# rlglab/minizero

Measured on AMD Instinct MI355X. Metric: self-play leaf-evals/s (9x9 Go AlphaZero n=400), higher is better.
Workload: dtype f32; 1 GPU; BASELINE configs[1]: 9x9 Go AlphaZero, n=400, 6 blocks x 64 ch, 256 parallel games per GPU, synthetic fixed-weight net (seed 0), Dirichlet noise + random rotation + softmax-count moves (reference defaults); games_per_gpu=256, actor_num_simulation=400, pipeline_lanes=1, backend=nccl

## Files before the change

### include/mzgpu.h

```cpp
#ifndef MZGPU_H
#define MZGPU_H
#include <stddef.h>
#include <stdint.h>

#ifdef __cplusplus
extern "C" {
#endif

#define MZ_OK 0
#define MZ_ERR_ARG (-1)
#define MZ_ERR_DEVICE (-2)
#define MZ_ERR_STATE (-3)
#define MZ_ERR_CAPACITY (-4)

#define MZ_HOST 0
#define MZ_DEVICE 1

const char* mz_last_error(void);
int mz_device_count(void);
int mz_usable_cpus(void);

typedef struct mz_net_desc {
    char game_name[64];
    int num_input_channels, input_channel_height, input_channel_width;
// ... 136 lines not shown
int mz_env_legal_mask(const mz_env* e, uint8_t* out);
int mz_env_features(const mz_env* e, int rotation, float* out);
int mz_env_action_from_string(const mz_env* e, const char* action_string);
int mz_env_feature_bits(const mz_env* e, int rotation, uint32_t* out);
int mz_env_name(const mz_env* e, char* out, int cap);

int mz_godev_playout(int device, int board_size, float komi, const int* actions, int count, int root_prefix, const int* rots,
                     uint32_t* feat_out, uint8_t* legal_out, int* terminal_out, float* eval_out, int* player_out);
int mz_envdev_playout(int device, const char* game, int board_size, float komi, const int* actions, int count, int root_prefix, const int* rots,
                      uint32_t* feat_out, uint8_t* legal_out, int* terminal_out, float* eval_out, int* player_out);
int mz_envdev_playout_conf(int device, const char* conf, const int* actions, int count, int root_prefix, const int* rots,
                           uint32_t* feat_out, uint8_t* legal_out, int* terminal_out, float* eval_out, int* player_out);
int mz_sort_candidates(int device, const float* policy, int n, int* order_out);
int mz_invert_values_device(int device, const float* values, int n, float* out);
int mz_exp_tanh_device(int device, const float* x, int n, float* exp_out, float* tanh_out);

#ifdef __cplusplus
}
#endif
#endif
```

### minizero_amd/__init__.py

```python
from .lib import (MzError, NetDesc, SearchCfg, WorkerStats, Net, Pool, Worker, Env, DataLoader, load, lib_path, make_desc,
                  param_count, generate_weights, device_count, usable_cpus, godev_playout, envdev_playout, envdev_playout_conf, sort_candidates, invert_values_device, exp_tanh_device, read_pt, read_weight_file, read_weights_once, weight_file_reads, DESCS, CONFIGS)
```

### minizero_amd/csrc/net.h

```cpp
#pragma once
#include "common.h"
#include "game_kind.h"
#include <string>

namespace mz {

struct ConvLayer {
    int cin, cin_pad, cout, cout_pad;
    size_t w_off, b_off;
    size_t w4_off;
    size_t wq_off;
    int cq;
};

struct HeadOffsets {
    int pc;
    size_t pconv_w, pconv_b, pfc_wT, pfc_b, vconv_w, vconv_b, vfc1_wT, vfc1_b, vfc2_w, vfc2_b;
};

struct DiscreteHeadOffsets {
    int hc = 0, hidden = 0, size = 0;
    size_t conv_w = 0, conv_b = 0, fc1_wT = 0, fc1_b = 0, fc2_wT = 0, fc2_b = 0;
};
struct AtariLayers {
// ... 40 lines not shown
    int reload(const float* raw, size_t n);

    int forwardAZ(const float* d_feat, int B, float* d_policy, float* d_logit, float* d_value, bool in_bits = false);
    bool hasFusedTower();
    int initial(const float* d_feat, int B, float* d_policy, float* d_logit, float* d_value, float* d_hidden, const int* d_dst_idx);
    int recurrent(const float* d_hidden_src, const int* d_src_idx, const float* d_action_planes, const int* d_action_ids, int B, float* d_policy,
                  float* d_logit, float* d_value, float* d_reward, float* d_hidden_dst, const int* d_dst_idx);
    int forwardAZ_any(const float* feat, int B, float* policy, float* logit, float* value, int where);
    int initial_any(const float* feat, int B, float* policy, float* logit, float* value, float* hidden, int where);
    int recurrent_any(const float* hidden_in, const float* action, int B, float* policy, float* logit, float* value, float* reward, float* hidden_out,
                      int where);
    int simLaunch(Pool& pool, const GoDevView& gv, float* d_policy, float* d_logit, float* d_value, const uint8_t* d_rot, int sim0, int nsims,
                  bool* launched, const float* d_root_noise = nullptr, float noise_eps = 0.0f, int noise_kind = kNoiseDirichlet, const struct GumbelView* gum = nullptr,
                  int* d_start = nullptr, bool host_start = false);
    void allowTailHelp(bool on) { tail_help_ = on; }
    bool hasSimKernel(int board_n, int env_kind = kGo, int num_simulation = 0) const;
    bool hasSimKernelWide(int board_n, int env_kind, int num_simulation) const;
    bool simWidePlan(int board_n, int env_kind, int num_simulation, const HeadParams& hp, int channels, int W32, size_t leaf_bytes, size_t scratch_bytes, int* lf, size_t* lds,
                     size_t* tile_bytes_out) const;
    int simLaunchWide(const struct SimArgs& a, const GoDevView& gv, int max_depth, const uint8_t* d_rot, int sim0, int nsims, bool host_start, int lf, size_t lds, bool* launched);
    int uploadSimArgs(const struct SimArgs& a);
    int simLaunchMz(Pool& pool, float* d_hidden, int slots, const unsigned* d_root_feat, const unsigned long long* d_root_legal, const int* d_root_turn,
                    int num_players, float* d_policy, float* d_logit, float* d_value, float* d_reward, int sim0, int nsims, bool* launched,
                    const float* d_root_noise, float noise_eps, int noise_kind, const GumbelView* gum, int* d_start, bool host_start, bool root_given = false,
                    int pre_epoch = 0, bool noise_applied = false, const SimMzMode& mode = SimMzMode());
    int simPreEvalMz(int games, int max_depth, int s0, int R, int epoch, bool* launched, bool want_alt = true, bool pairs = false);
    int simPreEvalBatchMz(int games, int max_depth, int s0, int R, int epoch, bool* launched, int force_nl = 0, bool want_alt = false);
    bool hasPreBatch() const;
    bool pairsAvailable() const { return pair_ok_; }
    void pairTrouble() { pair_ok_ = false; }
// ... 98 lines not shown
```

### minizero_amd/csrc/sim.hip

```cpp
#include "sim_az_body.h"
#include "sim_mz_body.h"

namespace mz {

MZ_SPEC_WAYS_IS(16);

template <int H, int W, int CIN0_PAD, int CDYN_PAD, int CPAD>
__global__ __launch_bounds__(512) void sim_kernel_mz(const SimArgs* __restrict__ a_, int sim0, int nsims, int host_start, int pre_epoch)
{
    CSimArgs* a = (CSimArgs*)a_;
    extern __shared__ __attribute__((aligned(16))) float tiles[];
    const int g = blockIdx.x, tid = threadIdx.x, lane = tid & 63, wave = tid >> 6;
    constexpr int CM = CIN0_PAD > CDYN_PAD ? (CIN0_PAD > CPAD ? CIN0_PAD : CPAD) : (CDYN_PAD > CPAD ? CDYN_PAD : CPAD);
    constexpr int kTileFloats = kTowerTiles * CM * planeStride(H, W);
    double* rcp_w = reinterpret_cast<double*>(tiles + kTileFloats);
    const int rcp_n = a->rcp_n;
    for (int i = tid; i < rcp_n; i += 512) { rcp_w[i] = a->pv.rcp_tab[i]; }
    LdsCDouble* rcp_lds = (LdsCDouble*)rcp_w;
    const int tab_n = rcp_n - 2;
    double* sqrt_w = rcp_w + rcp_n;
    float* bias_w = reinterpret_cast<float*>(sqrt_w + tab_n);
    int* spec_w = reinterpret_cast<int*>(bias_w + tab_n + (tab_n & 1));
    for (int i = tid; i < tab_n; i += 512) { sqrt_w[i] = a->pv.sqrt_tab[i]; bias_w[i] = a->pv.bias_tab[i]; }
    if (!a->atari) {
// ... 380 lines not shown
    X(8, 8, 4, 64, kRulesOthello)    \
    X(8, 8, 4, 8, kRulesOthello)     \
    X(3, 3, 4, 16, kRulesTicTacToe)

__global__ void sim_prof_fold(unsigned long long* tail)
{
    if (threadIdx.x != 0 || blockIdx.x != 0) { return; }
    const unsigned long long n = tail[5];
    if (n > 0) {
        const unsigned long long start = tail[0];
        tail[8] += 1;
        tail[9] += tail[1] - start;
        tail[10] += tail[2] - start;
        tail[11] += tail[3] / n - start;
        tail[12] += tail[6] / n;
    }
    tail[0] = ~0ull; tail[1] = ~0ull; tail[2] = 0; tail[3] = 0; tail[5] = 0; tail[6] = 0;
    tail[4] = wall_clock64();
}

int Net::simProfBuffer(int games, unsigned long long** prof)
{
    if (sim_prof_.n == 0) {
        if (!sim_prof_.alloc(size_t(games) * 8 + kSimProfTail)) { setError("hipMalloc of the profile buffer failed"); return MZ_ERR_DEVICE; }
        MZ_HIP(hipMemsetAsync(sim_prof_.p, 0, sim_prof_.n * sizeof(unsigned long long), stream_));
    }
    hipLaunchKernelGGL(sim_prof_fold, dim3(1), dim3(1), 0, stream_, sim_prof_.p + sim_prof_.n - kSimProfTail);
    MZ_HIP(hipGetLastError());
    *prof = sim_prof_.p;
    return MZ_OK;
}

// ... 83 lines not shown
    {
        double tw = 0, hd = 0;
        for (size_t g = 0; g < G; ++g) { tw += double(h[g * 8 + 1]); hd += double(h[g * 8 + 2]); }
        const double ran = std::max(1.0, sims_all - skipped);
        fprintf(stderr, "[mz sim prof] terminal leaves: network skipped in %.0f of %.0f simulations (%.2f %%; the game with the most: %.2f %%) -> per simulation that ran them: tower %.2f us, heads %.2f us\n",
                skipped, sims_all, 100.0 * skipped / std::max(1.0, sims_all), 100.0 * skipped_max, tw / ran * 0.01, hd / ran * 0.01);
    }
    fprintf(stderr, "[mz sim prof] value first: %llu of %.0f simulations in the new order; %llu walks arrived at the previous simulation's leaf, %llu waited there (avg %.2f us); "
                    "%llu waits at the join in front of the leaf\n",
            tail[16], sims_all, tail[17], tail[18], double(tail[19]) / std::max(1.0, double(tail[18])) * 0.01, tail[20]);
    if (tail[8] > 0) {
        const double L = double(tail[8]), first = double(tail[9]) / L * 0.01, last = double(tail[10]) / L * 0.01, mean = double(tail[11]) / L * 0.01;
        const double helping = double(tail[12]) / L * 0.01;
        fprintf(stderr, "[mz sim prof] launches: %llu, avg per launch from the first game's start: first game done %.1f us, mean %.1f us, last %.1f us -> %.1f %% of the CU time idles at the end of a launch\n",
                tail[8], first, mean, last, 100.0 * (last - mean - helping) / std::max(1e-9, last));
        if (tail[13] > 0 || tail[15] > 0) {
            double tw = 0;
            for (size_t g = 0; g < G; ++g) { tw += double(h[g * 8 + 1]); }
            const double ran = sims_all - skipped, pn = double(tail[13]), pt = double(tail[14]);
            fprintf(stderr, "[mz sim prof] tail help: %.0f of the %.0f simulations that ran the network had a pair tower (%.2f %%): tower %.2f us with a helper, %.2f us alone; %llu games helped, "
                            "a CU helps for %.1f us per launch after its own game (%.1f %% of the launch)\n",
                    pn, ran, 100.0 * pn / std::max(1.0, ran), pt / std::max(1.0, pn) * 0.01, (tw - pt) / std::max(1.0, ran - pn) * 0.01, tail[15], helping,
                    100.0 * helping / std::max(1e-9, last));
        }
    }
}

static size_t simLdsBound(size_t tile_bytes, int n, int A, size_t head_floats)
{
    const size_t rcp_n = size_t(n) + 5, max_depth = size_t(n) + 3;
    return tile_bytes + rcp_n * (2 * sizeof(double) + sizeof(float)) + kSpecWords * sizeof(int) + (size_t(5) * (A + 1) + 26 + 18 * 12 + 2 * max_depth + 2 + head_floats) * sizeof(float) +
           size_t(kGoSeenCap) * sizeof(uint64_t);
}

int Net::uploadSimArgs(const SimArgs& a)
{
    static_assert(sizeof(SimArgs) % 4 == 0, "SimArgs is copied as words");
    if (sim_args_host_.size() != sizeof(SimArgs) || memcmp(sim_args_host_.data(), &a, sizeof(SimArgs)) != 0) {
// ... 397 lines not shown
```

### minizero_amd/csrc/sim_az_body.h

```cpp
#pragma once
#include "net.h"
#ifdef MZ_SIM_TPROF
__device__ unsigned long long g_tp[64];
__shared__ unsigned long long s_tp_prev;
__shared__ int s_tp_idx;
#define MZ_TPROF(slot)                                                                         \
    do {                                                                                       \
        if ((slot) == 3 && threadIdx.x == 0 && blockIdx.x == 0) {                              \
            const unsigned long long t_ = clock64();                                           \
            g_tp[s_tp_idx & 63] += t_ - s_tp_prev; s_tp_prev = t_; ++s_tp_idx;                 \
        }                                                                                      \
    } while (0)
#endif
#ifdef MZ_SIM_HPROF
#ifndef MZ_HPROF_BLOCK
#define MZ_HPROF_BLOCK 0
#endif
__device__ unsigned long long g_hp[16];
__shared__ unsigned long long s_hp_prev;
#define MZ_HPROF(k)                                                                                   \
    do {                                                                                              \
        if (threadIdx.x == 0 && blockIdx.x == MZ_HPROF_BLOCK) {                                       \
            const unsigned long long t_ = wall_clock64();                                             \
            if ((k) > 0) { g_hp[(k)] += t_ - s_hp_prev; } else { g_hp[15] += 1; }                     \
// ... 396 lines not shown
}
template <int WPE, bool BIGA = false, bool FP = BIGA>
__device__ __noinline__ void simHeads(CSimArgs* __restrict__ a, int g, int tid, float* tiles, const float* xtile, int xcs, int xpw, float* xchg)
{
    simHeadsImpl<WPE, BIGA, FP>(a, g, tid, tiles, xtile, xcs, xpw, xchg);
}

__device__ __forceinline__ bool simLeafTerminal(CSimArgs* __restrict__ a, const float* xchg)
{
    if (a->no_spec & 16) { return false; }
    const int A = a->gv.A;
    const SimXchg x{A + (A & 1)};
    return __builtin_amdgcn_readfirstlane(reinterpret_cast<const int*>(xchg + x.scalars())[6]) != 0;
}

constexpr int kSimProfTail = 24;
__device__ __forceinline__ void simProfEnter(unsigned long long* tail)
{
    atomicMin(tail + 0, wall_clock64() - tail[4]);
}
__device__ __forceinline__ void simProfExit(unsigned long long* tail)
{
    const unsigned long long t = wall_clock64() - tail[4];
    atomicMin(tail + 1, t);
    atomicMax(tail + 2, t);
    atomicAdd(tail + 3, t);
    atomicAdd(tail + 5, 1ull);
}

template <int H, int W, int CIN0_PAD, int CPAD, bool BF = false>
constexpr int simWavesPerEu() { return (!BF && H * W <= 64 && kTowerTiles * (CIN0_PAD > CPAD ? CIN0_PAD : CPAD) * planeStride(H, W) * 4 <= 76 * 1024) ? 4 : 2; }
// ... 9 lines not shown
#endif
    g = __builtin_amdgcn_readfirstlane(g);
    const GoDevView gv = simLeafView(ldc(&a->gv), xchg, g);
    return towerBody<H, W, CIN0_PAD, CPAD>(reinterpret_cast<const float*>(gv.feat), a->params, *(const TowerArgs*)&a->ta, nullptr, g, tid, tiles);
}

template <int H, int W>
__device__ __noinline__ const float* simTowerBf16(CSimArgs* __restrict__ a, int g, int tid, float* tiles, float* xchg)
{
    g = __builtin_amdgcn_readfirstlane(g);
    const GoDevView gv = simLeafView(ldc(&a->gv), xchg, g);
    return towerBodyBf16<H, W>(reinterpret_cast<const unsigned*>(gv.feat), a->wfrag, a->params, *(const TowerArgsBf16*)&a->tb, nullptr, g, tid,
                               reinterpret_cast<char*>(tiles));
}

template <int H, int W, int CIN0_PAD, int CPAD>
__device__ __noinline__ const float* simTowerPair(CSimArgs* __restrict__ a, int g, int tid, float* tiles, float* xchg, int seq, unsigned xseq, int* abort_lds)
{
    g = __builtin_amdgcn_readfirstlane(g);
    seq = __builtin_amdgcn_readfirstlane(seq);
    xseq = __builtin_amdgcn_readfirstlane(xseq);
    const GoDevView gv = simLeafView(ldc(&a->gv), xchg, g);
    const unsigned* bits = reinterpret_cast<const unsigned*>(gv.feat) + size_t(g) * gv.channels * gv.W32;
    unsigned* hb = a->help + size_t(g) * a->help_words;
    const int fw = gv.channels * gv.W32;
    if (tid < helpCmdUnits(fw)) {
        hpu4 u;
        u.x = bits[3 * tid];
        u.y = 3 * tid + 1 < fw ? bits[3 * tid + 1] : 0u;
        u.z = 3 * tid + 2 < fw ? bits[3 * tid + 2] : 0u;
        u.w = unsigned(seq);
        asm volatile("global_store_dwordx4 %0, %1, off" ::"v"(hb + kHpCmd + 4 * tid), "v"(u) : "memory");
    }
    HelpCtx c{hb, 0, xseq, abort_lds, a->err};
    return towerBodyPair<H, W, CIN0_PAD, CPAD>(bits, a->params, *(const TowerArgs*)&a->ta, tid, tiles, c);
}

template <int H, int W, int CIN0_PAD, int CPAD>
__device__ __noinline__ void simHelpTail(CSimArgs* __restrict__ a, int g, int tid, float* tiles, unsigned* bits, int nsims, int* s_help)
{
    g = __builtin_amdgcn_readfirstlane(g);
    nsims = __builtin_amdgcn_readfirstlane(nsims);
    const int lane = tid & 63, wave = __builtin_amdgcn_readfirstlane(tid >> 6);
    const int games = gridDim.x, words = a->help_words, min_left = a->help_min_left;
    const int fw = a->gv.channels * a->gv.W32, units = helpCmdUnits(fw);
    const unsigned myxcc = hpXccId();
    unsigned long long* ptail = a->prof ? a->prof + size_t(games) * 8 : nullptr;
    for (int round = 0; round < 64; ++round) {
        if (wave == 0) {
            unsigned key = ~0u;
            for (int o = (g & 7) + 8 * lane; o < games; o += 8 * 64) {
                const unsigned* ob = a->help + size_t(o) * words;
                const unsigned x = hpLoadU(ob + kHpXcc), p = hpLoadU(ob + kHpProgress), h = hpLoadU(ob + kHpHelper);
                const unsigned k = (p << 10) | unsigned(o);
                if (o != g && x == myxcc && h == 0u && int(p) + min_left <= nsims && k < key) { key = k; }
            }
            for (int o = 32; o > 0; o >>= 1) { const unsigned k2 = __shfl_xor(key, o); key = k2 < key ? k2 : key; }
            if (lane == 0) {
                int cl = 0;
                if (key != ~0u) {
                    unsigned expected = 0u;
                    unsigned* hw = a->help + size_t(key & 1023u) * words + kHpHelper;
                    cl = __hip_atomic_compare_exchange_strong(hw, &expected, unsigned(g) + 1u, __ATOMIC_RELAXED, __ATOMIC_RELAXED, __HIP_MEMORY_SCOPE_AGENT) ? int(key & 1023u) + 1 : -1;
                }
                s_help[1] = cl;
                s_help[2] = int(key >> 10);
            }
        }
        __syncthreads();
        const int cl = __builtin_amdgcn_readfirstlane(s_help[1]);
        unsigned last = unsigned(__builtin_amdgcn_readfirstlane(s_help[2]));
        __syncthreads();
        if (cl == 0) { return; }
        if (cl < 0) { continue; }
        const unsigned long long th0 = ptail ? wall_clock64() : 0;
        unsigned* ob = a->help + size_t(cl - 1) * words;
        HelpCtx c{ob, 1, 0u, s_help, a->err};
        for (;;) {
            if (wave == 0) {
                int st = 0;
                hpu4 u;
                for (int i = 0; i < kHpPollLimit && st == 0; ++i) {
                    const unsigned* src = ob + kHpCmd + 4 * (lane < units ? lane : 0);
                    asm volatile("global_load_dwordx4 %0, %1, off sc1\n\ts_waitcnt vmcnt(0)" : "=v"(u) : "v"(src) : "memory");
                    const unsigned sq = __builtin_amdgcn_readfirstlane(u.w);
                    if (__all(u.w == sq) && sq > last && sq <= unsigned(nsims)) { st = 1; last = sq; }
                    else if (hpLoadU(ob + kHpProgress) >= unsigned(nsims)) { st = 2; }
                    else { __builtin_amdgcn_s_sleep(4); }
                }
                if (st == 1 && lane < units) {
                    bits[3 * lane] = u.x;
                    if (3 * lane + 1 < fw) { bits[3 * lane + 1] = u.y; }
                    if (3 * lane + 2 < fw) { bits[3 * lane + 2] = u.z; }
                }
                if (lane == 0) {
                    if (st == 0) { atomicExch(a->err, 96); }
                    s_help[1] = st;
                }
            }
            __syncthreads();
            const int st = __builtin_amdgcn_readfirstlane(s_help[1]);
            if (st != 1) {
                if (ptail && tid == 0) { atomicAdd(ptail + 6, wall_clock64() - th0); atomicAdd(ptail + 15, 1ull); }
                if (st == 0) { return; }
                break;
            }
            if (!towerBodyPair<H, W, CIN0_PAD, CPAD>(bits, a->params, *(const TowerArgs*)&a->ta, tid, tiles, c)) { return; }
            __syncthreads();
        }
        __syncthreads();
    }
}

template <int H, int W, int CIN0_PAD, int CPAD, int CPL, bool BF = false>
__global__ __launch_bounds__(512) __attribute__((amdgpu_waves_per_eu(simWavesPerEu<H, W, CIN0_PAD, CPAD, BF>(), 4))) void sim_kernel(const SimArgs* __restrict__ a_, const uint8_t* __restrict__ rot_tab, int sim0, int nsims, int host_start)
{
    CSimArgs* a = (CSimArgs*)a_;
    extern __shared__ __attribute__((aligned(16))) float tiles[];
    const int g = blockIdx.x, tid = threadIdx.x, lane = tid & 63, wave = tid >> 6;
    const int games = gridDim.x;
    constexpr int WPE = simWavesPerEu<H, W, CIN0_PAD, CPAD, BF>();
    constexpr int kTileFloats = simTileFloats<H, W, CIN0_PAD, CPAD, BF>();
// ... 33 lines not shown
            uint64_t* zk = leaf_smem + goLeafKeyWord(a->gv.Ppad, a->gv.W, a->pv.max_depth);
            for (int i = tid; i < 2 * a->gv.P; i += 512) { zk[i] = a->gv.key[i]; }
            __syncthreads();
        }
    }
    unsigned long long* prof = a->prof ? a->prof + size_t(g) * 8 : nullptr;
    int* const node_count = reinterpret_cast<int*>(xchg) - 1;
    if (tid == 0) { *node_count = a->pv.num_nodes[g]; }
    if (prof && tid == 0) { simProfEnter(a->prof + size_t(games) * 8); }
    constexpr bool kHelp = !BF && WPE == 2 && CPL > 0 && pairTowerShape<H, W, CPAD>();
    __shared__ int s_help[kHelp ? kVfWords : 4];
    const bool help_on = kHelp && (host_start & 2) != 0;
    unsigned* const help_blk = help_on ? a->help + size_t(g) * a->help_words : nullptr;
    unsigned help_xseq = 0;
    unsigned long long pair_n = 0, pair_t = 0;
    if (help_on && tid == 0) { s_help[0] = 0; s_help[1] = 0; hpStoreU(help_blk + kHpXcc, hpXccId()); }
    bool vf = false;
    if constexpr (kHelp) {
        vf = leaf_smem != nullptr && !a->use_gumbel && !a->pv.value_rescale && a->cand_coop != 2 && !(a->no_spec & 64);
        if (tid >= kVfBackup && tid < kVfWords) { s_help[tid] = 0; }
    }
    unsigned long long vf_t0 = 0, vf_n = 0;
    __syncthreads();
    for (int s = 0; s < nsims; ++s) {
        const int slot = sim0 + s;
        const int rot = rot_tab[size_t(s) * games + g];
        unsigned long long t0 = 0, t1 = 0, t2 = 0, t3 = 0, t4 = 0;
        if (prof) { t0 = (vf && s > 0) ? vf_t0 : wall_clock64(); }
        if (kHelp && vf) {
            if constexpr (kHelp) {
                if (wave == 0) {
                    if (s == 0) {
                        if (slot == 1 && a->root_noise) { simApplyRootNoise<WPE>(a, g, lane); }
                        simWalkVf(a, g, lane, rcp_lds, spec, xchg, (a->no_spec & 2) ? 0 : 1, -1, 0, s_help);
                    } else {
                        const bool waited = vfWait((LdsI32*)s_help + kVfExpand, s, a->err, lane);
                        if (prof && waited && lane == 0) { s_help[kVfStats + 3] += 1; }
                        if (help_on && lane == 0) { hpStoreU(help_blk + kHpProgress, unsigned(s)); }
                    }
                    simLeafVf<CPL>(a, rot, slot, g, lane, xchg, seen_lds, leaf_smem, s_help);
                } else if (s == 0 && wave <= kHelpSegs && spec.w && !(a->no_spec & 2)) {
                    simSelectHelper(a, g, lane, wave, 1, rcp_lds, spec);
                } else if (help_on && tid == 7 * 64) {
                    s_help[1] = int(hpLoadU(help_blk + kHpHelper));
                }
            }
        } else if (wave == 0) {
            if (slot == 1 && a->root_noise) { simApplyRootNoise<WPE>(a, g, lane); }
            if (a->use_gumbel) { simGumbelStart<WPE>(a, slot, s == 0 && (host_start & 1) != 0, g, lane, tiles); }
            simSelectLeaf<CPL, WPE>(a, rot, slot, g, lane, tiles, rcp_lds, spec, xchg, seen_lds, (a->no_spec & 2) ? 0 : s + 1, leaf_smem);
        } else if (WPE == 2 && wave <= kHelpSegs && spec.w && !(a->no_spec & 2)) {
            simSelectHelper(a, g, lane, wave, s + 1, rcp_lds, spec);
        } else if (kHelp && help_on && tid == 7 * 64) {
            s_help[1] = int(hpLoadU(help_blk + kHpHelper));
        }
        __syncthreads();
        const bool pair = kHelp && help_on && __builtin_amdgcn_readfirstlane(s_help[1]) != 0;
        const bool term = simLeafTerminal(a, xchg);
        if constexpr (CPL > 0) {
            if (!term) {
                simLeafPlanes<CPL>(a, rot, g, wave, lane, leaf_smem ? leaf_smem : reinterpret_cast<const uint64_t*>(tiles), xchg);
                __syncthreads();
            }
        }
        if (prof) { t1 = wall_clock64(); }
        const float* xt = nullptr;
        if (!term) {
            if constexpr (BF) { xt = simTowerBf16<H, W>(a, g, tid, tiles, xchg); }
            else if constexpr (WPE == 4) {
                const GoDevView gvt = simLeafView(ldc(&a->gv), xchg, g);
                xt = towerBody<H, W, CIN0_PAD, CPAD>(reinterpret_cast<const float*>(gvt.feat), a->params, *(const TowerArgs*)&a->ta, nullptr, g, tid, tiles);
            }
            else if constexpr (kHelp) {
                if (pair) {
                    xt = simTowerPair<H, W, CIN0_PAD, CPAD>(a, g, tid, tiles, xchg, s + 1, help_xseq, s_help);
                    if (!xt) { return; }
                    help_xseq += unsigned(a->ta.nlayers);
                }
                else { xt = simTower<H, W, CIN0_PAD, CPAD>(a, g, tid, tiles, xchg); }
            }
            else { xt = simTower<H, W, CIN0_PAD, CPAD>(a, g, tid, tiles, xchg); }
        }
        __syncthreads();
        if (prof) { t2 = wall_clock64(); }
        if constexpr (WPE == 4) { if (!term) { simHeadsImpl<WPE>(a, g, tid, tiles, xt, planeStride(H, W), W + 2, xchg); } }
        else if (leaf_smem && wave >= 6) { simLeafRest<CPL>(a, rot, slot, g, lane, xchg, seen_lds, leaf_smem, 7 - wave); }
        else if (!term) { simHeads<WPE, false, (MZ_HEADS_FP != 0)>(a, g, tid, tiles, xt, planeStride(H, W), W + 2, xchg); }
        else if (leaf_smem) { __syncthreads(); __syncthreads(); }
        __syncthreads();
        if (prof) { t3 = wall_clock64(); }
        if (kHelp && vf) {
            if constexpr (kHelp) {
                const bool more = s + 1 < nsims;
                if (wave == 0) {
                    simBackupOnly<WPE>(a, slot, g, lane, tiles, xchg);
                    vfPublish((LdsI32*)s_help + kVfBackup, s + 1, lane);
                    if (prof && tid == 0) {
                        t4 = wall_clock64();
                        prof[0] += t1 - t0 + (term ? t3 - t1 : 0); prof[1] += term ? 0 : t2 - t1; prof[2] += term ? 0 : t3 - t2; prof[3] += t4 - t3;
                        prof[4] += 1 + (static_cast<unsigned long long>(term) << 32);
                        if (pair && !term) { pair_n += 1; pair_t += t2 - t1; }
                        vf_n += 1;
                    }
                    vf_t0 = t4;
                    if (more) {
                        if (slot + 1 == 1 && a->root_noise) {
                            vfWait((LdsI32*)s_help + kVfExpand, s + 1, a->err, lane);
                            simApplyRootNoise<WPE>(a, g, lane);
                        }
                        simWalkVf(a, g, lane, rcp_lds, spec, xchg, (a->no_spec & 2) ? 0 : s + 2, __builtin_amdgcn_readfirstlane(s_help[kVfLeaf]), s + 1, s_help);
                    }
                } else if (wave <= kHelpSegs) {
                    if (more && spec.w && !(a->no_spec & 2)) {
                        vfWait((LdsI32*)s_help + kVfBackup, s + 1, a->err, lane);
                        simSelectHelper(a, g, lane, wave, s + 2, rcp_lds, spec);
                    }
// ... 10 lines not shown
            const SimXchg x{A + (A & 1)};
            if (a->cand_coop) { simCandRank(A, reinterpret_cast<const int*>(xchg + x.scalars())[1], wave, lane, tiles); }
        }
        __syncthreads();
        {
            const bool split = !a->pv.value_rescale;
            if (wave == 0) { simCandExpand<WPE>(a, rot, slot, g, lane, tiles, xchg, split ? 1 : 0); }
            else if (wave == 1 && split) { simBackupOnly<WPE>(a, slot, g, lane, tiles, xchg); }
        }
        __syncthreads();
        if (prof && tid == 0) {
            t4 = wall_clock64();
            prof[0] += t1 - t0 + (term ? t3 - t1 : 0); prof[1] += term ? 0 : t2 - t1; prof[2] += term ? 0 : t3 - t2; prof[3] += t4 - t3;
            prof[4] += 1 + (static_cast<unsigned long long>(term) << 32);
            if (pair && !term) { pair_n += 1; pair_t += t2 - t1; }
        }
        if (kHelp && help_on && tid == 0) { hpStoreU(help_blk + kHpProgress, unsigned(s) + 1u); }
    }
    if constexpr (kHelp) {
        if (vf) {
            __syncthreads();
            if (help_on && tid == 0) { hpStoreU(help_blk + kHpProgress, unsigned(nsims)); }
            if (prof && tid == 0) {
                unsigned long long* ptail = a->prof + size_t(games) * 8;
                atomicAdd(ptail + 16, vf_n);
                for (int i = 0; i < 4; ++i) { atomicAdd(ptail + 17 + i, static_cast<unsigned long long>(s_help[kVfStats + i])); }
            }
        }
    }
    if (tid == 0) { a->pv.num_nodes[g] = *node_count; }
    if (prof && tid == 0) {
        simProfExit(a->prof + size_t(games) * 8);
        if (pair_n) { atomicAdd(a->prof + size_t(games) * 8 + 13, pair_n); atomicAdd(a->prof + size_t(games) * 8 + 14, pair_t); }
    }
    if (prof && tid == 0 && spec_w) {
        prof[7] += (static_cast<unsigned long long>(spec_w[kSpecWays * kSpecWay + 1]) << 40) | (static_cast<unsigned long long>(spec_w[kSpecWays * kSpecWay + 5]) << 20) | spec_w[kSpecWays * kSpecWay + 3];
        prof[6] += static_cast<unsigned long long>(spec_w[kSpecWays * kSpecWay + 7]) << 40;
    }
    if constexpr (kHelp) {
        if (help_on) {
            const int A = a->gv.A;
            const SimXchg x{A + (A & 1)};
            __syncthreads();
            simHelpTail<H, W, CIN0_PAD, CPAD>(a, g, tid, tiles, reinterpret_cast<unsigned*>(xchg + x.feat()), nsims, s_help);
        }
    }
}

// ... 3 lines not shown
```

### minizero_amd/csrc/sim_help.h

```cpp
#pragma once
#include "net_body.h"

namespace mz {

constexpr int kHpXcc = 0;
constexpr int kHpProgress = 1;
constexpr int kHpHelper = 32;
constexpr int kHpCmd = 64;
constexpr int kHpXbuf = 320;
constexpr int kHpPollLimit = 1 << 21;
constexpr int kHpMaxUnits = 64;
typedef unsigned hpu4 __attribute__((ext_vector_type(4)));
inline size_t helpWords(int C, int P) { return (size_t(kHpXbuf) + 2 * size_t(C) * P + 31) / 32 * 32; }
__host__ __device__ constexpr int helpCmdUnits(int feat_words) { return (feat_words + 2) / 3; }

__device__ __forceinline__ unsigned hpLoadU(const unsigned* p) { return __hip_atomic_load(p, __ATOMIC_RELAXED, __HIP_MEMORY_SCOPE_AGENT); }
__device__ __forceinline__ float hpLoadF(const float* p) { return __uint_as_float(__hip_atomic_load(reinterpret_cast<const unsigned*>(p), __ATOMIC_RELAXED, __HIP_MEMORY_SCOPE_AGENT)); }
__device__ __forceinline__ void hpStoreU(unsigned* p, unsigned v) { __hip_atomic_store(p, v, __ATOMIC_RELAXED, __HIP_MEMORY_SCOPE_AGENT); }
__device__ __forceinline__ unsigned hpXccId()
{
    unsigned id;
    asm volatile("s_getreg_b32 %0, hwreg(HW_REG_XCC_ID)" : "=s"(id));
    return (id & 15u) + 1u;
}

struct HelpCtx {
// ... 99 lines not shown
    }
    __syncthreads();
    const int simd = wave & 3, ot = 2 * c.member + (simd >> 1), grp = simd & 1;
    bool ok;
    if (wave < 4) {
        ok = pairRun<H, W, CIN0_PAD, CPAD, 2, false>(params, ta, T0, T1, lane, tid, ot, 3 * grp, c);
    } else {
        __builtin_amdgcn_s_setprio(2);
        if (grp == 0) { ok = pairRun<H, W, CIN0_PAD, CPAD, 1, false>(params, ta, T0, T1, lane, tid, ot, 2, c); }
        else { ok = pairRun<H, W, CIN0_PAD, CPAD, 1, true>(params, ta, T0, T1, lane, tid, ot, 5, c); }
        __builtin_amdgcn_s_setprio(0);
    }
    return ok ? T1 : nullptr;
}

}
```

### minizero_amd/lib.py

```python
import ctypes as C
import os

import numpy as np

_HERE = os.path.dirname(os.path.abspath(__file__))
_LIB = None

MZ_HOST, MZ_DEVICE = 0, 1


class MzError(RuntimeError):
    pass


def lib_path():
    return os.environ.get("MZ_LIBMZGPU") or os.path.join(_HERE, "libmzgpu.so")


class NetDesc(C.Structure):
    _fields_ = [("game_name", C.c_char * 64),
                ("num_input_channels", C.c_int), ("input_channel_height", C.c_int), ("input_channel_width", C.c_int),
                ("num_hidden_channels", C.c_int), ("hidden_channel_height", C.c_int), ("hidden_channel_width", C.c_int),
                ("num_action_feature_channels", C.c_int), ("num_blocks", C.c_int), ("action_size", C.c_int),
                ("num_value_hidden_channels", C.c_int), ("discrete_value_size", C.c_int), ("type", C.c_int)]
# ... 608 lines not shown
    L = load()
    v = np.ascontiguousarray(values, np.float32)
    out = np.zeros(len(v), np.float32)
    _check(L, L.mz_invert_values_device(device, _f(v), len(v), _f(out)))
    return out


def exp_tanh_device(x, device=0):
    L = load()
    v = np.ascontiguousarray(x, np.float32)
    e, t = np.zeros(len(v), np.float32), np.zeros(len(v), np.float32)
    _check(L, L.mz_exp_tanh_device(device, _f(v), len(v), _f(e), _f(t)))
    return e, t


def sort_candidates(policy, device=0):
    L = load()
    p = np.ascontiguousarray(policy, np.float32)
    order = np.zeros(len(p), np.int32)
    _check(L, L.mz_sort_candidates(device, _f(p), len(p), _i(order)))
    return order
```

Measured before the change: 1.638 million leaf-evals/s.

## Add quad-member tail-help towers so three idle CUs can assist a game

Extends the tail-help scheme so that a game already paired with one helper can recruit two more helper workgroups on the same XCD. Together they split the residual tower into four oc-tile members, exchanging partial activations through global memory. The goal is to cut the idle CU time at the end of a launch, when only a few games are still running. In exchange it adds more cross-CU polling and synchronisation and reuses the exchange buffer in a new layout. It also packs mode and xseq into the command word, adds profiling counters, and adds a test entry point.

```diff
diff --git a/include/mzgpu.h b/include/mzgpu.h
--- a/include/mzgpu.h
+++ b/include/mzgpu.h
@@ -174,6 +174,7 @@
 int mz_sort_candidates(int device, const float* policy, int n, int* order_out);
 int mz_invert_values_device(int device, const float* values, int n, float* out);
 int mz_exp_tanh_device(int device, const float* x, int n, float* exp_out, float* tanh_out);
+int mz_tail_towers_device(mz_net* net, const uint32_t* bits, int towers, int members, float* out, uint32_t* xcc_out, int* err_flag_out, int* status_out);
 
 #ifdef __cplusplus
 }
diff --git a/minizero_amd/__init__.py b/minizero_amd/__init__.py
--- a/minizero_amd/__init__.py
+++ b/minizero_amd/__init__.py
@@ -1,2 +1,2 @@
 from .lib import (MzError, NetDesc, SearchCfg, WorkerStats, Net, Pool, Worker, Env, DataLoader, load, lib_path, make_desc,
-                  param_count, generate_weights, device_count, usable_cpus, godev_playout, envdev_playout, envdev_playout_conf, sort_candidates, invert_values_device, exp_tanh_device, read_pt, read_weight_file, read_weights_once, weight_file_reads, DESCS, CONFIGS)
+                  param_count, generate_weights, device_count, usable_cpus, godev_playout, envdev_playout, envdev_playout_conf, sort_candidates, invert_values_device, exp_tanh_device, tail_towers, read_pt, read_weight_file, read_weights_once, weight_file_reads, DESCS, CONFIGS)
diff --git a/minizero_amd/csrc/net.h b/minizero_amd/csrc/net.h
--- a/minizero_amd/csrc/net.h
+++ b/minizero_amd/csrc/net.h
@@ -78,6 +78,7 @@
                   bool* launched, const float* d_root_noise = nullptr, float noise_eps = 0.0f, int noise_kind = kNoiseDirichlet, const struct GumbelView* gum = nullptr,
                   int* d_start = nullptr, bool host_start = false);
     void allowTailHelp(bool on) { tail_help_ = on; }
+    int tailTowers(const unsigned* bits, int towers, int members, float* out, unsigned* xcc, int* err_flag, int* status);
     bool hasSimKernel(int board_n, int env_kind = kGo, int num_simulation = 0) const;
     bool hasSimKernelWide(int board_n, int env_kind, int num_simulation) const;
     bool simWidePlan(int board_n, int env_kind, int num_simulation, const HeadParams& hp, int channels, int W32, size_t leaf_bytes, size_t scratch_bytes, int* lf, size_t* lds,
diff --git a/minizero_amd/csrc/sim.hip b/minizero_amd/csrc/sim.hip
--- a/minizero_amd/csrc/sim.hip
+++ b/minizero_amd/csrc/sim.hip
@@ -418,8 +418,13 @@
         tail[10] += tail[2] - start;
         tail[11] += tail[3] / n - start;
         tail[12] += tail[6] / n;
+        for (int c = 0; c < 3; ++c) {
+            const unsigned long long end = tail[24 + c] * tail[2];
+            tail[30 + c] += (end > tail[27 + c] ? end - tail[27 + c] : 0) / n;
+        }
     }
     tail[0] = ~0ull; tail[1] = ~0ull; tail[2] = 0; tail[3] = 0; tail[5] = 0; tail[6] = 0;
+    for (int c = 24; c < 30; ++c) { tail[c] = 0; }
     tail[4] = wall_clock64();
 }
 
@@ -533,14 +538,21 @@
         const double helping = double(tail[12]) / L * 0.01;
         fprintf(stderr, "[mz sim prof] launches: %llu, avg per launch from the first game's start: first game done %.1f us, mean %.1f us, last %.1f us -> %.1f %% of the CU time idles at the end of a launch\n",
                 tail[8], first, mean, last, 100.0 * (last - mean - helping) / std::max(1e-9, last));
-        if (tail[13] > 0 || tail[15] > 0) {
+        if (tail[13] > 0 || tail[15] > 0 || tail[21] > 0) {
             double tw = 0;
             for (size_t g = 0; g < G; ++g) { tw += double(h[g * 8 + 1]); }
-            const double ran = sims_all - skipped, pn = double(tail[13]), pt = double(tail[14]);
+            const double ran = sims_all - skipped, qn = double(tail[21]), qt = double(tail[22]), pn = double(tail[13]) + qn, pt = double(tail[14]) + qt;
             fprintf(stderr, "[mz sim prof] tail help: %.0f of the %.0f simulations that ran the network had a pair tower (%.2f %%): tower %.2f us with a helper, %.2f us alone; %llu games helped, "
                             "a CU helps for %.1f us per launch after its own game (%.1f %% of the launch)\n",
                     pn, ran, 100.0 * pn / std::max(1.0, ran), pt / std::max(1.0, pn) * 0.01, (tw - pt) / std::max(1.0, ran - pn) * 0.01, tail[15], helping,
                     100.0 * helping / std::max(1e-9, last));
+            fprintf(stderr, "[mz sim prof] tail help, quad towers: %.0f of the %.0f simulations that ran the network had a quad tower (%.2f %%): tower %.2f us with three helpers, %.2f us with "
+                            "one; %llu games went from pair to quad towers\n",
+                    qn, ran, 100.0 * qn / std::max(1.0, ran), qt / std::max(1.0, qn) * 0.01, (pt - qt) / std::max(1.0, pn - qn) * 0.01, tail[23]);
+            const double ia = double(tail[30]) / L * 0.01, ib = double(tail[31]) / L * 0.01, ic = double(tail[32]) / L * 0.01;
+            fprintf(stderr, "[mz sim prof] tail help, idle CU time by the reason the CU stopped looking for a game to help (%% of the launch): (a) every running game of its XCD had its "
+                            "helpers %.2f %%, (b) no game of its XCD was running any more %.2f %%, (c) only games with fewer than help_min_left simulations were left %.2f %%\n",
+                    100.0 * ia / std::max(1e-9, last), 100.0 * ib / std::max(1e-9, last), 100.0 * ic / std::max(1e-9, last));
         }
     }
 }
diff --git a/minizero_amd/csrc/sim_az_body.h b/minizero_amd/csrc/sim_az_body.h
--- a/minizero_amd/csrc/sim_az_body.h
+++ b/minizero_amd/csrc/sim_az_body.h
@@ -434,7 +434,7 @@
     return __builtin_amdgcn_readfirstlane(reinterpret_cast<const int*>(xchg + x.scalars())[6]) != 0;
 }
 
-constexpr int kSimProfTail = 24;
+constexpr int kSimProfTail = 40;
 __device__ __forceinline__ void simProfEnter(unsigned long long* tail)
 {
     atomicMin(tail + 0, wall_clock64() - tail[4]);
@@ -474,8 +474,8 @@
                                reinterpret_cast<char*>(tiles));
 }
 
-template <int H, int W, int CIN0_PAD, int CPAD>
-__device__ __noinline__ const float* simTowerPair(CSimArgs* __restrict__ a, int g, int tid, float* tiles, float* xchg, int seq, unsigned xseq, int* abort_lds)
+template <int H, int W, int CIN0_PAD, int CPAD, int MODE>
+__device__ __forceinline__ const float* simTowerHelped(CSimArgs* __restrict__ a, int g, int tid, float* tiles, float* xchg, int seq, unsigned xseq, int* abort_lds)
 {
     g = __builtin_amdgcn_readfirstlane(g);
     seq = __builtin_amdgcn_readfirstlane(seq);
@@ -489,11 +489,40 @@
         u.x = bits[3 * tid];
         u.y = 3 * tid + 1 < fw ? bits[3 * tid + 1] : 0u;
         u.z = 3 * tid + 2 < fw ? bits[3 * tid + 2] : 0u;
-        u.w = unsigned(seq);
+        u.w = hpCmdWord(unsigned(seq), MODE, xseq);
         asm volatile("global_store_dwordx4 %0, %1, off" ::"v"(hb + kHpCmd + 4 * tid), "v"(u) : "memory");
     }
     HelpCtx c{hb, 0, xseq, abort_lds, a->err};
-    return towerBodyPair<H, W, CIN0_PAD, CPAD>(bits, a->params, *(const TowerArgs*)&a->ta, tid, tiles, c);
+    if constexpr (MODE == kHpModeQuad) { return towerBodyQuad<H, W, CIN0_PAD, CPAD>(bits, a->params, *(const TowerArgs*)&a->ta, tid, tiles, c); }
+    else { return towerBodyPair<H, W, CIN0_PAD, CPAD>(bits, a->params, *(const TowerArgs*)&a->ta, tid, tiles, c); }
+}
+template <int H, int W, int CIN0_PAD, int CPAD>
+__device__ __noinline__ const float* simTowerPair(CSimArgs* __restrict__ a, int g, int tid, float* tiles, float* xchg, int seq, unsigned xseq, int* abort_lds)
+{
+    return simTowerHelped<H, W, CIN0_PAD, CPAD, kHpModePair>(a, g, tid, tiles, xchg, seq, xseq, abort_lds);
+}
+template <int H, int W, int CIN0_PAD, int CPAD>
+__device__ __noinline__ const float* simTowerQuad(CSimArgs* __restrict__ a, int g, int tid, float* tiles, float* xchg, int seq, unsigned xseq, int* abort_lds)
+{
+    return simTowerHelped<H, W, CIN0_PAD, CPAD, kHpModeQuad>(a, g, tid, tiles, xchg, seq, xseq, abort_lds);
+}
+
+__device__ __forceinline__ int simHelpMode(const unsigned* help_blk)
+{
+    if (hpLoadU(help_blk + kHpHelper) == 0u) { return 0; }
+    const unsigned h2 = hpLoadU(help_blk + kHpHelper2), h3 = hpLoadU(help_blk + kHpHelper3);
+    return (h2 != 0u && h3 != 0u) ? 2 : 1;
+}
+
+template <int H, int W, int CIN0_PAD, int CPAD, int MODE>
+__device__ __noinline__ bool simHelpTower(CSimArgs* __restrict__ a, int o, int member, unsigned xseq, int tid, float* tiles, const unsigned* bits, int* abort_lds)
+{
+    o = __builtin_amdgcn_readfirstlane(o);
+    member = __builtin_amdgcn_readfirstlane(member);
+    xseq = __builtin_amdgcn_readfirstlane(xseq);
+    HelpCtx c{a->help + size_t(o) * a->help_words, member, xseq, abort_lds, a->err};
+    if constexpr (MODE == kHpModeQuad) { return towerBodyQuad<H, W, CIN0_PAD, CPAD>(bits, a->params, *(const TowerArgs*)&a->ta, tid, tiles, c) != nullptr; }
+    else { return towerBodyPair<H, W, CIN0_PAD, CPAD>(bits, a->params, *(const TowerArgs*)&a->ta, tid, tiles, c) != nullptr; }
 }
 
 template <int H, int W, int CIN0_PAD, int CPAD>
@@ -504,38 +533,61 @@
     const int lane = tid & 63, wave = __builtin_amdgcn_readfirstlane(tid >> 6);
     const int games = gridDim.x, words = a->help_words, min_left = a->help_min_left;
     const int fw = a->gv.channels * a->gv.W32, units = helpCmdUnits(fw);
+    const bool more_slots = !(a->no_spec & 128);
     const unsigned myxcc = hpXccId();
     unsigned long long* ptail = a->prof ? a->prof + size_t(games) * 8 : nullptr;
     for (int round = 0; round < 64; ++round) {
         if (wave == 0) {
-            unsigned key = ~0u;
+            unsigned key = ~0u, key2 = ~0u;
+            bool enough = false, running = false;
             for (int o = (g & 7) + 8 * lane; o < games; o += 8 * 64) {
                 const unsigned* ob = a->help + size_t(o) * words;
                 const unsigned x = hpLoadU(ob + kHpXcc), p = hpLoadU(ob + kHpProgress), h = hpLoadU(ob + kHpHelper);
+                const unsigned h2 = hpLoadU(ob + kHpHelper2), h3 = hpLoadU(ob + kHpHelper3);
                 const unsigned k = (p << 10) | unsigned(o);
-                if (o != g && x == myxcc && h == 0u && int(p) + min_left <= nsims && k < key) { key = k; }
+                const bool mine = o != g && x == myxcc, left = int(p) + min_left <= nsims;
+                running = running || (mine && int(p) < nsims);
+                enough = enough || (mine && left);
+                if (mine && left && h == 0u && k < key) { key = k; }
+                if (mine && left && more_slots && h != 0u && (h2 == 0u || h3 == 0u) && k < key2) { key2 = k; }
             }
             for (int o = 32; o > 0; o >>= 1) { const unsigned k2 = __shfl_xor(key, o); key = k2 < key ? k2 : key; }
+            for (int o = 32; o > 0; o >>= 1) { const unsigned k2 = __shfl_xor(key2, o); key2 = k2 < key2 ? k2 : key2; }
+            enough = __any(enough);
+            running = __any(running);
             if (lane == 0) {
-                int cl = 0;
+                int cl = 0, slot = 1;
                 if (key != ~0u) {
                     unsigned expected = 0u;
                     unsigned* hw = a->help + size_t(key & 1023u) * words + kHpHelper;
                     cl = __hip_atomic_compare_exchange_strong(hw, &expected, unsigned(g) + 1u, __ATOMIC_RELAXED, __ATOMIC_RELAXED, __HIP_MEMORY_SCOPE_AGENT) ? int(key & 1023u) + 1 : -1;
+                } else if (key2 != ~0u) {
+                    key = key2;
+                    unsigned* hw = a->help + size_t(key & 1023u) * words;
+                    cl = -1;
+                    for (slot = 2; slot <= 3 && cl < 0; ++slot) {
+                        unsigned expected = 0u;
+                        if (__hip_atomic_compare_exchange_strong(hw + (slot == 2 ? kHpHelper2 : kHpHelper3), &expected, unsigned(g) + 1u, __ATOMIC_RELAXED, __ATOMIC_RELAXED,
+                                                                 __HIP_MEMORY_SCOPE_AGENT)) { cl = int(key & 1023u) + 1; break; }
+                    }
                 }
                 s_help[1] = cl;
-                s_help[2] = int(key >> 10);
+                s_help[2] = cl != 0 ? int(key >> 10) : (enough ? 0 : running ? 2 : 1);
+                s_help[3] = slot;
             }
         }
         __syncthreads();
         const int cl = __builtin_amdgcn_readfirstlane(s_help[1]);
         unsigned last = unsigned(__builtin_amdgcn_readfirstlane(s_help[2]));
-        __syncthreads();
-        if (cl == 0) { return; }
+        const int slot = __builtin_amdgcn_readfirstlane(s_help[3]);
+        __syncthreads();
+        if (cl == 0) {
+            if (ptail && tid == 0) { atomicAdd(ptail + 24 + last, 1ull); atomicAdd(ptail + 27 + last, wall_clock64() - ptail[4]); }
+            return;
+        }
         if (cl < 0) { continue; }
         const unsigned long long th0 = ptail ? wall_clock64() : 0;
         unsigned* ob = a->help + size_t(cl - 1) * words;
-        HelpCtx c{ob, 1, 0u, s_help, a->err};
         for (;;) {
             if (wave == 0) {
                 int st = 0;
@@ -543,29 +595,34 @@
                 for (int i = 0; i < kHpPollLimit && st == 0; ++i) {
                     const unsigned* src = ob + kHpCmd + 4 * (lane < units ? lane : 0);
                     asm volatile("global_load_dwordx4 %0, %1, off sc1\n\ts_waitcnt vmcnt(0)" : "=v"(u) : "v"(src) : "memory");
-                    const unsigned sq = __builtin_amdgcn_readfirstlane(u.w);
-                    if (__all(u.w == sq) && sq > last && sq <= unsigned(nsims)) { st = 1; last = sq; }
-                    else if (hpLoadU(ob + kHpProgress) >= unsigned(nsims)) { st = 2; }
+                    const unsigned cw = __builtin_amdgcn_readfirstlane(u.w), sq = hpCmdSeq(cw);
+                    if (__all(u.w == cw) && sq > last && sq <= unsigned(nsims)) {
+                        last = sq;
+                        if (slot == 1 || hpCmdMode(cw) == kHpModeQuad) { st = 1 + hpCmdMode(cw); s_help[2] = int(hpCmdXseq(cw)); }
+                    }
+                    else if (hpLoadU(ob + kHpProgress) >= unsigned(nsims)) { st = 3; }
                     else { __builtin_amdgcn_s_sleep(4); }
                 }
-                if (st == 1 && lane < units) {
+                if ((st == 1 || st == 2) && lane < units) {
                     bits[3 * lane] = u.x;
                     if (3 * lane + 1 < fw) { bits[3 * lane + 1] = u.y; }
                     if (3 * lane + 2 < fw) { bits[3 * lane + 2] = u.z; }
                 }
                 if (lane == 0) {
-                    if (st == 0) { atomicExch(a->err, 96); }
+                    if (st == 0) { atomicExch(a->err, slot == 1 ? 96 : kHpErrQuadCmd); }
                     s_help[1] = st;
                 }
             }
             __syncthreads();
             const int st = __builtin_amdgcn_readfirstlane(s_help[1]);
-            if (st != 1) {
+            if (st != 1 && st != 2) {
                 if (ptail && tid == 0) { atomicAdd(ptail + 6, wall_clock64() - th0); atomicAdd(ptail + 15, 1ull); }
                 if (st == 0) { return; }
                 break;
             }
-            if (!towerBodyPair<H, W, CIN0_PAD, CPAD>(bits, a->params, *(const TowerArgs*)&a->ta, tid, tiles, c)) { return; }
+            const unsigned xseq = unsigned(__builtin_amdgcn_readfirstlane(s_help[2]));
+            if (!(st == 2 ? simHelpTower<H, W, CIN0_PAD, CPAD, kHpModeQuad>(a, cl - 1, slot, xseq, tid, tiles, bits, s_help)
+                          : simHelpTower<H, W, CIN0_PAD, CPAD, kHpModePair>(a, cl - 1, 1, xseq, tid, tiles, bits, s_help))) { return; }
             __syncthreads();
         }
         __syncthreads();
@@ -629,6 +686,7 @@
     unsigned* const help_blk = help_on ? a->help + size_t(g) * a->help_words : nullptr;
     unsigned help_xseq = 0;
     unsigned long long pair_n = 0, pair_t = 0;
+    unsigned long long quad_n = 0, quad_t = 0;
     if (help_on && tid == 0) { s_help[0] = 0; s_help[1] = 0; hpStoreU(help_blk + kHpXcc, hpXccId()); }
     bool vf = false;
     if constexpr (kHelp) {
@@ -657,7 +715,7 @@
                 } else if (s == 0 && wave <= kHelpSegs && spec.w && !(a->no_spec & 2)) {
                     simSelectHelper(a, g, lane, wave, 1, rcp_lds, spec);
                 } else if (help_on && tid == 7 * 64) {
-                    s_help[1] = int(hpLoadU(help_blk + kHpHelper));
+                    s_help[1] = simHelpMode(help_blk);
                 }
             }
         } else if (wave == 0) {
@@ -667,10 +725,11 @@
         } else if (WPE == 2 && wave <= kHelpSegs && spec.w && !(a->no_spec & 2)) {
             simSelectHelper(a, g, lane, wave, s + 1, rcp_lds, spec);
         } else if (kHelp && help_on && tid == 7 * 64) {
-            s_help[1] = int(hpLoadU(help_blk + kHpHelper));
-        }
-        __syncthreads();
-        const bool pair = kHelp && help_on && __builtin_amdgcn_readfirstlane(s_help[1]) != 0;
+            s_help[1] = simHelpMode(help_blk);
+        }
+        __syncthreads();
+        const int help_mode = (kHelp && help_on) ? __builtin_amdgcn_readfirstlane(s_help[1]) : 0;
+        const bool pair = help_mode == 1, quad = help_mode == 2;
         const bool term = simLeafTerminal(a, xchg);
         if constexpr (CPL > 0) {
             if (!term) {
@@ -689,6 +748,11 @@
             else if constexpr (kHelp) {
                 if (pair) {
                     xt = simTowerPair<H, W, CIN0_PAD, CPAD>(a, g, tid, tiles, xchg, s + 1, help_xseq, s_help);
+                    if (!xt) { return; }
+                    help_xseq += unsigned(a->ta.nlayers);
+                }
+                else if (quad) {
+                    xt = simTowerQuad<H, W, CIN0_PAD, CPAD>(a, g, tid, tiles, xchg, s + 1, help_xseq, s_help);
                     if (!xt) { return; }
                     help_xseq += unsigned(a->ta.nlayers);
                 }
@@ -715,6 +779,7 @@
                         prof[0] += t1 - t0 + (term ? t3 - t1 : 0); prof[1] += term ? 0 : t2 - t1; prof[2] += term ? 0 : t3 - t2; prof[3] += t4 - t3;
                         prof[4] += 1 + (static_cast<unsigned long long>(term) << 32);
                         if (pair && !term) { pair_n += 1; pair_t += t2 - t1; }
+                        if (quad && !term) { quad_n += 1; quad_t += t2 - t1; }
                         vf_n += 1;
                     }
                     vf_t0 = t4;
@@ -755,6 +820,7 @@
             prof[0] += t1 - t0 + (term ? t3 - t1 : 0); prof[1] += term ? 0 : t2 - t1; prof[2] += term ? 0 : t3 - t2; prof[3] += t4 - t3;
             prof[4] += 1 + (static_cast<unsigned long long>(term) << 32);
             if (pair && !term) { pair_n += 1; pair_t += t2 - t1; }
+            if (quad && !term) { quad_n += 1; quad_t += t2 - t1; }
         }
         if (kHelp && help_on && tid == 0) { hpStoreU(help_blk + kHpProgress, unsigned(s) + 1u); }
     }
@@ -773,6 +839,7 @@
     if (prof && tid == 0) {
         simProfExit(a->prof + size_t(games) * 8);
         if (pair_n) { atomicAdd(a->prof + size_t(games) * 8 + 13, pair_n); atomicAdd(a->prof + size_t(games) * 8 + 14, pair_t); }
+        if (quad_n) { atomicAdd(a->prof + size_t(games) * 8 + 21, quad_n); atomicAdd(a->prof + size_t(games) * 8 + 22, quad_t); atomicAdd(a->prof + size_t(games) * 8 + 23, pair_n ? 1ull : 0ull); }
     }
     if (prof && tid == 0 && spec_w) {
         prof[7] += (static_cast<unsigned long long>(spec_w[kSpecWays * kSpecWay + 1]) << 40) | (static_cast<unsigned long long>(spec_w[kSpecWays * kSpecWay + 5]) << 20) | spec_w[kSpecWays * kSpecWay + 3];
diff --git a/minizero_amd/csrc/sim_help.h b/minizero_amd/csrc/sim_help.h
--- a/minizero_amd/csrc/sim_help.h
+++ b/minizero_amd/csrc/sim_help.h
@@ -7,9 +7,17 @@
 constexpr int kHpProgress = 1;
 constexpr int kHpHelper = 32;
 constexpr int kHpCmd = 64;
+constexpr int kHpHelper2 = 192;
+constexpr int kHpHelper3 = 224;
 constexpr int kHpXbuf = 320;
 constexpr int kHpPollLimit = 1 << 21;
-constexpr int kHpMaxUnits = 64;
+constexpr int kHpMaxUnits = 32;
+constexpr int kHpErrQuad = 98, kHpErrQuadCmd = 99;
+constexpr int kHpModePair = 0, kHpModeQuad = 1;
+__host__ __device__ constexpr unsigned hpCmdWord(unsigned seq, int mode, unsigned xseq) { return (seq & 0x0FFFFFFFu) | (unsigned(mode) << 28) | ((xseq & 3u) << 29); }
+__host__ __device__ constexpr unsigned hpCmdSeq(unsigned w) { return w & 0x0FFFFFFFu; }
+__host__ __device__ constexpr int hpCmdMode(unsigned w) { return int((w >> 28) & 1u); }
+__host__ __device__ constexpr unsigned hpCmdXseq(unsigned w) { return w >> 29; }
 typedef unsigned hpu4 __attribute__((ext_vector_type(4)));
 inline size_t helpWords(int C, int P) { return (size_t(kHpXbuf) + 2 * size_t(C) * P + 31) / 32 * 32; }
 __host__ __device__ constexpr int helpCmdUnits(int feat_words) { return (feat_words + 2) / 3; }
@@ -139,4 +147,104 @@
     return ok ? T1 : nullptr;
 }
 
-}
+template <int H, int W, int CPAD>
+__device__ __forceinline__ bool hpExchangeQuad(HelpCtx& c, float* __restrict__ tout, int tid, bool read)
+{
+    constexpr int P = H * W, PW = W + 2, CS = planeStride(H, W), OWN = CPAD / 4 * P, OTHERS = 3 * OWN;
+    const unsigned sign = hpSign(c);
+    const float* xb = reinterpret_cast<const float*>(c.hb + kHpXbuf) + size_t(c.xseq & 1) * CPAD * P;
+    const int own0 = c.member * OWN;
+    ++c.xseq;
+    __syncthreads();
+    if (!read) { return true; }
+    constexpr int K = (OTHERS + 511) / 512;
+    unsigned got[K];
+    bool ok = false;
+    for (int polls = 0; polls < kHpPollLimit; ++polls) {
+        ok = true;
+#pragma unroll
+        for (int j = 0; j < K; ++j) {
+            const int i = tid + j * 512;
+            const bool want = i < OTHERS;
+            const int src = want ? i + (i >= own0 ? OWN : 0) : (own0 == 0 ? OWN : 0);
+            got[j] = __float_as_uint(hpLoadF(xb + src));
+            ok = ok && (!want || (got[j] & 0x80000000u) == sign);
+        }
+        ok = __all(ok);
+        if (ok) { break; }
+        __builtin_amdgcn_s_sleep(2);
+    }
+    if (!ok && (tid & 63) == 0) { *c.abort_lds = 1; atomicExch(c.err, kHpErrQuad); }
+#pragma unroll
+    for (int j = 0; j < K; ++j) {
+        const int i = tid + j * 512;
+        if (i < OTHERS) {
+            const int src = i + (i >= own0 ? OWN : 0), ch = src / P, p = src % P;
+            tout[ch * CS + (p / W + 1) * PW + (p % W) + 1] = __uint_as_float(got[j] & 0x7FFFFFFFu);
+        }
+    }
+    __syncthreads();
+    return *c.abort_lds == 0;
+}
+
+template <int H, int W, int CIN0_PAD, int CPAD, bool HAS_TILE, bool CORNER>
+__device__ __forceinline__ bool quadRun(const float* __restrict__ params, const TowerArgs& ta, float* __restrict__ T0, float* __restrict__ T1, int lane, int tid, int tile, HelpCtx& c)
+{
+    constexpr int P = H * W;
+    const int ot = c.member;
+    const PixSet<1> px = makePixSet<H, W, 1>(lane, HAS_TILE ? tile : 0);
+    float aS[CIN0_PAD / 4], aA[CPAD / 4], aB[CPAD / 4];
+    bool have = false;
+    if (ta.has_stem) {
+        const float* nw = ta.nlayers > 1 ? params + ta.w_off[1] : nullptr;
+        if constexpr (HAS_TILE) {
+            tower_layer<H, W, CIN0_PAD / 4, 1, CPAD / 4, CORNER, false, true>(T0, nullptr, T1, nullptr, params + ta.w_off[0], params + ta.b_off[0], ta.C, ta.OT, lane, ot, px, false,
+                                                                              aS, nw, aA, hpPart<CPAD, P>(c, ot), hpSign(c));
+        }
+        have = nw != nullptr;
+        if (!hpExchangeQuad<H, W, CPAD>(c, T1, tid, c.member == 0 || ta.nlayers > 1)) { return false; }
+    }
+    float *x = T1, *tmp = T0;
+#pragma unroll 1
+    for (int l = ta.has_stem; l < ta.nlayers; ++l) {
+        const bool second = ((l - ta.has_stem) & 1) != 0, last = l + 1 == ta.nlayers;
+        if constexpr (HAS_TILE) {
+            tower_layer<H, W, CPAD / 4, 1, CPAD / 4, CORNER, false, true>(second ? tmp : x, second ? x : nullptr, second ? x : tmp, nullptr, params + ta.w_off[l], params + ta.b_off[l],
+                                                                          ta.C, ta.OT, lane, ot, px, have, aA, last ? nullptr : params + ta.w_off[l + 1], aB, hpPart<CPAD, P>(c, ot),
+                                                                          hpSign(c));
+#pragma unroll
+            for (int cg = 0; cg < CPAD / 4; ++cg) { aA[cg] = aB[cg]; }
+        }
+        have = !last;
+        if (!hpExchangeQuad<H, W, CPAD>(c, second ? x : tmp, tid, c.member == 0 || !last)) { return false; }
+    }
+    return true;
+}
+
+template <int H, int W, int CIN0_PAD, int CPAD>
+__device__ __forceinline__ float* towerBodyQuad(const unsigned* __restrict__ bits, const float* __restrict__ params, const TowerArgs& ta, int tid, float* __restrict__ tiles,
+                                                HelpCtx& c)
+{
+    static_assert(pairTowerShape<H, W, CPAD>(), "quad tower: one oc-tile per member, pixel tiles {0, 1}, {2, 3}, {4}, {corner}");
+    constexpr int P = H * W, PW = W + 2, CS = planeStride(H, W), W32 = (P + 31) / 32;
+    constexpr int CMAX = CIN0_PAD > CPAD ? CIN0_PAD : CPAD;
+    const int lane = tid & 63, wave = tid >> 6;
+    float* T0 = tiles;
+    float* T1 = tiles + CMAX * CS;
+    for (int i = tid; i < kTowerTiles * CMAX * CS / 4; i += 512) { reinterpret_cast<float4*>(tiles)[i] = make_float4(0.0f, 0.0f, 0.0f, 0.0f); }
+    __syncthreads();
+    float* Tin = ta.has_stem ? T0 : T1;
+    for (int i = tid; i < ta.cin0 * P; i += 512) {
+        const int ch = i / P, p = i - ch * P;
+        Tin[ch * CS + (p / W + 1) * PW + (p % W) + 1] = ((bits[ch * W32 + (p >> 5)] >> (p & 31)) & 1u) ? 1.0f : 0.0f;
+    }
+    __syncthreads();
+    bool ok;
+    if (wave == 3) { ok = quadRun<H, W, CIN0_PAD, CPAD, true, true>(params, ta, T0, T1, lane, tid, 5, c); }
+    else if (wave < 3) { ok = quadRun<H, W, CIN0_PAD, CPAD, true, false>(params, ta, T0, T1, lane, tid, 2 * wave, c); }
+    else if (wave < 6) { ok = quadRun<H, W, CIN0_PAD, CPAD, true, false>(params, ta, T0, T1, lane, tid, 2 * (wave - 4) + 1, c); }
+    else { ok = quadRun<H, W, CIN0_PAD, CPAD, false, false>(params, ta, T0, T1, lane, tid, 0, c); }
+    return ok ? T1 : nullptr;
+}
+
+}
diff --git a/minizero_amd/lib.py b/minizero_amd/lib.py
--- a/minizero_amd/lib.py
+++ b/minizero_amd/lib.py
@@ -646,6 +646,19 @@
     return e, t
 
 
+def tail_towers(net, bits, members):
+    L = load()
+    L.mz_tail_towers_device.argtypes = [C.c_void_p, C.POINTER(C.c_uint32), C.c_int, C.c_int, C.POINTER(C.c_float), C.POINTER(C.c_uint32), C.POINTER(C.c_int), C.POINTER(C.c_int)]
+    b = np.ascontiguousarray(bits, np.uint32)
+    T = b.shape[0]
+    out = np.zeros((T, 64, 81), np.float32)
+    xcc = np.zeros((members, T), np.uint32)
+    err, status = C.c_int(0), C.c_int(0)
+    _check(L, L.mz_tail_towers_device(net.h, b.ctypes.data_as(C.POINTER(C.c_uint32)), T, members, _f(out), xcc.ctypes.data_as(C.POINTER(C.c_uint32)),
+                                      C.byref(err), C.byref(status)))
+    return out, xcc, err.value, status.value
+
+
 def sort_candidates(policy, device=0):
     L = load()
     p = np.ascontiguousarray(policy, np.float32)
```

Result: faster. 1.677 million leaf-evals/s (median of 6 runs) (+2.3%).
